# emanuele-artioli/elvis

Measured on AMD Instinct MI355X. Metric: restored 1080p frames/sec, SinSR 4x path (ELVIS v2 Downsample), higher is better.
Workload: dtype f16; 1 GPU; 30-frame 1920x1080 synthetic clip per GPU, ELVIS v2 Downsample (SinSR 4x), block 8, levels 0-3, weights seed 0 (random init), quantize=True; frames_per_gpu=30, parallelism=single GPU, gn_fused_into_conv=True, frames_per_invocation=15

## Files before the change

elvis_amd/csrc/conv.hip:

```cpp
#include "conv_kernels.inc"
#include "conv_ws.inc"
#include <string.h>

__attribute__((visibility("hidden"))) int elvis_conv_launch_f32_(const void* conv_args, int halo, int tco, int id, hipStream_t stream, void* query);
__attribute__((visibility("hidden"))) int elvis_conv_pack_x3p_(const float* w_oihw, void* packed, int cout, int ctot, int nkc, int n_co_tiles,
                                                              int tco, int taps, hipStream_t stream);

#include <atomic>
static std::atomic<int> g_no_halo{0};
static bool no_halo() { return g_no_halo.load(std::memory_order_relaxed) > 0; }
extern "C" int elvis_conv_debug_set(const char* key, int value) {
    ELVIS_REQUIRE(key, "elvis_conv_debug_set: null key");
    if (!strcmp(key, "no_halo")) { g_no_halo.store(value, std::memory_order_relaxed); return ELVIS_OK; }
    ELVIS_REQUIRE(false, "elvis_conv_debug_set: unknown key '%s'", key);
}

static void conv_geom(const elvis_conv_desc* d, int* nkc1, int* nkc, int* co_pad) {
    int kc = kc_of(d);
    *nkc1 = (d->cin + kc - 1) / kc;
    *nkc = *nkc1 + (d->cin2 > 0 ? (d->cin2 + kc - 1) / kc : 0);
    TileCfg t = choose_tile(d->cout);
    *co_pad = ((d->cout + t.tco - 1) / t.tco) * t.tco;
}

extern "C" size_t elvis_conv_packed_weight_bytes(const elvis_conv_desc* d) {
    if (!d || d->cin <= 0 || d->cout <= 0) return 0;
    int nkc1, nkc, co_pad;
    conv_geom(d, &nkc1, &nkc, &co_pad);
    return (size_t)d->ksize * d->ksize * nkc * co_pad * (x3_planar_fmt(d) ? 128 : 64);
}

extern "C" int elvis_conv_pack_weights(const elvis_conv_desc* d, const float* w_oihw, void* packed,
                                       elvis_stream_t stream) {
    int rc = validate(d);
    if (rc) return rc;
    ELVIS_REQUIRE(w_oihw && packed, "elvis_conv_pack_weights: null pointer");
    int nkc1, nkc, co_pad;
    conv_geom(d, &nkc1, &nkc, &co_pad);
    if (x3_planar_fmt(d)) {
        const int tco = choose_tile(d->cout).tco;
        return elvis_conv_pack_x3p_(w_oihw, packed, d->cout, d->cin + d->cin2, nkc, co_pad / tco, tco, d->ksize * d->ksize, (hipStream_t)stream);
    }
    int KC = kc_elems(d->dtype);
    long long total = (long long)d->ksize * d->ksize * nkc * co_pad * KC;
    int grid = (int)((total + 255) / 256);
    int ctot = d->cin + d->cin2;
    const int tco_ = choose_tile(d->cout).tco, wco = tco_ >= 64 ? 4 : tco_ / 16;
    if (d->dtype == ELVIS_F16)
        hipLaunchKernelGGL(pack_weights_kernel<half_t>, dim3(grid), dim3(256), 0, (hipStream_t)stream, w_oihw,
                           (half_t*)packed, d->cout, ctot, d->ksize, nkc, co_pad, KC, total, wco);
    else
        hipLaunchKernelGGL(pack_weights_kernel<float>, dim3(grid), dim3(256), 0, (hipStream_t)stream, w_oihw,
                           (float*)packed, d->cout, ctot, d->ksize, nkc, co_pad, KC, total, wco, d->dtype == ELVIS_F32X3 ? 1 : 0);
    ELVIS_CHECK_LAUNCH("elvis_conv_pack_weights");
    return ELVIS_OK;
}

static bool x3_eligible(const elvis_conv_desc* d) {
    if (!(d->dtype == ELVIS_F32X3 && halo_eligible(d) && !no_halo() && choose_tile(d->cout).tco >= 64)) return false;
    return !x3_planar_fmt(d) || x3_planar_run(d);
}
extern "C" int elvis_conv_x3_eligible(const elvis_conv_desc* d) {
    if (!d || validate(d)) return 0;
    return x3_eligible(d) ? 1 : 0;
}

enum class ConvPath { WS, HALO, IGEMM };
static ConvPath conv_path(const elvis_conv_desc* d, bool has_residual, bool has_stats) {
    if (no_halo()) return ConvPath::IGEMM;
    if (ws_shape_ok(d) && !has_residual && !has_stats) return ConvPath::WS;
    return halo_eligible(d) ? ConvPath::HALO : ConvPath::IGEMM;
}

static int conv_walk(const elvis_conv_desc* d, ConvPath path, const ConvArgs& a, hipStream_t stream, ConvPick* query) {
    const TileCfg t = choose_tile(d->cout);
    const bool f16 = d->dtype == ELVIS_F16;
    if (path == ConvPath::WS) return dispatch_ws(a, t.tco, stream, query);
    if (path == ConvPath::IGEMM) return f16 ? dispatch<half_t>(a, t.id, stream, query) : elvis_conv_launch_f32_(&a, 0, t.tco, t.id, stream, query);
    if (!f16) return elvis_conv_launch_f32_(&a, 1, t.tco, t.id, stream, query);
    switch (t.tco) {
        case 128: return launch_halo<half_t, 128>(a, stream, query);
        case 64: return launch_halo<half_t, 64>(a, stream, query);
        case 32: return launch_halo<half_t, 32>(a, stream, query);
        default: return launch_halo<half_t, 16>(a, stream, query);
    }
}

static int conv_plan(const elvis_conv_desc* d, ConvPath path, ConvArgs& a, ConvPick& pick) {
    a.n = d->n; a.h = d->h; a.w_in = d->w;
    a.cin = d->cin; a.cin_pitch = d->cin_pitch; a.cin2 = d->cin2; a.cin2_pitch = d->cin2_pitch;
    a.cout = d->cout; a.cout_pitch = d->cout_pitch;
    a.ksize = d->ksize; a.stride = d->stride; a.pad = d->pad_before; a.upsample = d->upsample;
    a.ho = d->ho; a.wo = d->wo; a.act = d->act; a.prologue = d->prologue;
    conv_geom(d, &a.nkc1, &a.nkc, &a.co_pad);
    TileCfg t = choose_tile(d->cout);
    a.M = (long long)d->n * d->ho * d->wo;
    a.n_co_tiles = a.co_pad / t.tco;
    a.n_px_tiles = (a.M + t.tpx - 1) / t.tpx;
    const bool s2d = d->ksize == 2 && d->subpixel == ELVIS_CONV_S2D;
    const bool subpix = d->ksize == 2 && !s2d;
    a.sub = d->ksize == 2;
    a.par_a = subpix ? (d->subpixel - 1) >> 1 : 0;
    a.par_b = subpix ? (d->subpixel - 1) & 1 : 0;
    a.ostr = subpix ? 2 : 1;
    a.pad2y = subpix ? 1 - a.par_a : (s2d ? d->pad_before : 0);
    a.pad2x = subpix ? 1 - a.par_b : (s2d ? d->pad_before : 0);
    a.s2d = s2d ? 1 : 0;
    a.istr = s2d ? 2 : 1;
    a.nkc_c = s2d ? d->cin / 4 / kc_of(d) : 0x3fffffff;
    a.wfull = d->w;
    if (s2d) {
        a.h = d->ho;
        a.w_in = d->wo;
    }
    a.x3 = d->dtype == ELVIS_F32X3 ? (x3_planar_run(d) ? 2 : 1) : 0;
    a.two = (halo_two(d) || halo_g1(d)) ? 1 : 0;
    a.tall = (halo_two(d) && halo_tall(d)) ? 1 : 0;
    int rc = conv_walk(d, path, a, nullptr, &pick);
    if (rc) return rc;
    a.tiles_x = ((subpix ? d->w : d->wo) + HALO_TX - 1) / HALO_TX;
    a.tiles_y = pick.ty > 0 ? ((subpix ? d->h : d->ho) + pick.ty - 1) / pick.ty : 0;
    a.strip = HALO_STRIP < a.tiles_x ? HALO_STRIP : 0;
    a.strip_full = a.strip > 0 ? a.tiles_x / a.strip : 0;
    return ELVIS_OK;
}

extern "C" int elvis_conv_stats_tiles(const elvis_conv_desc* d) {
    if (!d || !halo_eligible(d)) return 0;
    ConvArgs a{};
    ConvPick pick{};
    if (conv_plan(d, ConvPath::HALO, a, pick)) return 0;
    return d->n * a.tiles_y * a.tiles_x;
}

extern "C" int elvis_conv_kernel_name_for_call(const elvis_conv_desc* d, int has_residual, int has_stats, char* buf, size_t n) {
    int rc = validate(d);
    if (rc) return rc;
    ELVIS_REQUIRE(buf && n > 0, "elvis_conv_kernel_name: null buffer");
    ConvArgs a{};
    ConvPick pick{};
    rc = conv_plan(d, conv_path(d, has_residual != 0, has_stats != 0), a, pick);
    if (rc) return rc;
    snprintf(buf, n, "%s", pick.name);
    return ELVIS_OK;
}

extern "C" int elvis_conv_kernel_name(const elvis_conv_desc* d, char* buf, size_t n) {
    return elvis_conv_kernel_name_for_call(d, 0, 0, buf, n);
}

extern "C" int elvis_conv2d(const elvis_conv_desc* d, const void* x, const void* x2, const void* w_packed,
                            const float* bias, const void* residual, int residual_pitch, const float* pa,
                            const float* pb, void* out, float* stats, elvis_stream_t stream) {
    int rc = validate(d);
    if (rc) return rc;
    ELVIS_REQUIRE(x && w_packed && out, "elvis_conv2d: null pointer");
    ELVIS_REQUIRE(d->cin2 == 0 || x2, "elvis_conv2d: cin2 > 0 but x2 is null");
    ELVIS_REQUIRE(!d->prologue || (pa && pb), "elvis_conv2d: prologue requested without pa/pb");
    ELVIS_REQUIRE(d->dtype != ELVIS_F32X3 || x3_eligible(d),
                  "elvis_conv2d: this shape has no compensated-f16 kernel (elvis_conv_x3_eligible): run it as ELVIS_F32");
    ELVIS_REQUIRE(!residual || residual_pitch >= d->cout, "elvis_conv2d: bad residual pitch");
    ELVIS_REQUIRE(((uintptr_t)x | (uintptr_t)(x2 ? x2 : x) | (uintptr_t)w_packed | (uintptr_t)out) % 16 == 0,
                  "elvis_conv2d: pointers must be 16-byte aligned");
    const ConvPath path = conv_path(d, residual != nullptr, stats != nullptr);
    ELVIS_REQUIRE(path != ConvPath::IGEMM || !stats, "elvis_conv2d: fused statistics need a 3x3/stride-1 conv with cout >= 64 (query elvis_conv_stats_tiles)");
    ELVIS_REQUIRE(path == ConvPath::IGEMM || (long long)d->n * d->h * d->w < 0x7fffffffLL, "conv: input too large for 32-bit pixel indices");
    ConvArgs a{};
    ConvPick pick{};
    rc = conv_plan(d, path, a, pick);
    if (rc) return rc;
    a.x = x; a.x2 = x2; a.w = w_packed; a.bias = bias; a.res = residual; a.pa = pa; a.pb = pb; a.out = out;
    a.res_pitch = residual_pitch; a.stats = stats;
    return conv_walk(d, path, a, (hipStream_t)stream, nullptr);
}
```

elvis_amd/csrc/conv_kernels.inc:

```
#pragma once
#include "common.h"

#ifndef ELVIS_CONV_HOOKS
#define ELVIS_STAGE(x) x
#define ELVIS_STAGE_W(x) x
#define ELVIS_STAGE_H(x) x
#define ELVIS_SETPRIO(x)
#define ELVIS_BARRIER() __syncthreads()
#define ELVIS_HOOK_SKIP_STORE(tv)
#define ELVIS_HOOK_STAMP_BEGIN
#define ELVIS_HOOK_STAMP_LOOP
#define ELVIS_HOOK_STAMP_EPILOGUE
#define ELVIS_HOOK_STAMP_END
#endif

namespace {

struct ConvArgs {
    const void* x;
    const void* x2;
    const void* w;
    const float* bias;
    const void* res;
    const float* pa;
// ... 486 lines not shown
    int h_src[H_PER];
    unsigned h_ok = 0;
#pragma unroll
    for (int i = 0; i < H_PER; ++i) {
        int chunk = tid + i * NT;
        int pix = chunk >> 2;
        int hy = pix / HX, hx = pix - hy * HX;
        int gy = oy0 + hy - pad_y, gx = ox0 + hx - pad_x;
        bool ok = chunk < HCH && gy >= 0 && gy < lh && gx >= 0 && gx < lw;
        int sy = p.upsample ? (gy >> 1) : gy, sx = p.upsample ? (gx >> 1) : gx;
        h_src[i] = ok ? ((nimg * p.h + sy) * p.istr * p.w_in + sx) * p.istr : 0;
        h_ok |= (ok ? 1u : 0u) << i;
    }
    const bool halo_inside = oy0 - pad_y >= 0 && oy0 - pad_y + HY <= lh && ox0 - pad_x >= 0 && ox0 - pad_x + HX <= lw &&
                             (p.cin % KC) == 0 && (p.cin2 % KC) == 0 && p.cin_pitch >= p.nkc1 * KC && !(KS == 2 && p.s2d);
    const int q4 = tid & 3;
    const int nkc = p.nkc;
    const int nrows = nkc * KS;

    constexpr int HA = (H_PER + 1) / 2;
    uint4 hreg[H_PER];

    int wl_off[W_PER];
#pragma unroll
    for (int i = 0; i < W_PER; ++i) {
        int chunk = tid + i * NT;
        wl_off[i] = lds_row_off(chunk >> 2, chunk & 3);
    }

    auto chunk_c0 = [&](int kc, int& pixoff) -> int {
        pixoff = 0;
        if (KS == 2 && p.s2d) {
            const int ph = kc / p.nkc_c;
            pixoff = (ph >> 1) * p.wfull + (ph & 1);
            return (kc - ph * p.nkc_c) * KC + q4 * VEC;
        }
        return (kc >= p.nkc1 ? kc - p.nkc1 : kc) * KC + q4 * VEC;
    };
    auto halo_load = [&](int kc, int i0, int i1, bool live = true) {
        const bool second = kc >= p.nkc1;
        const char* xsrc = (const char*)(second ? p.x2 : p.x);
        const int pitch = second ? p.cin2_pitch : p.cin_pitch;
        int pixoff;
        const int c0 = chunk_c0(kc, pixoff);
        const int c0c = c0 < pitch ? c0 : 0;
        const long long lv = live ? (long long)sizeof(T) : 0;
#pragma unroll
        for (int i = i0; i < i1; ++i)
            hreg[i] = *reinterpret_cast<const uint4*>(xsrc + ((long long)(h_src[i] + pixoff) * pitch + c0c) * lv);
    };
    auto halo_store = [&](int kc, int buf, int i0, int i1) {
        const bool second = kc >= p.nkc1;
        const int pitch = second ? p.cin2_pitch : p.cin_pitch;
        int pixoff_;
        const int c0 = chunk_c0(kc, pixoff_);
        const bool ch_ok = c0 < pitch;
        char* dst = halo + buf * HALO_BYTES;
        float la[VEC], lb[VEC];
        if (PRO) {
            const float* tp = ptab + (kc * 4 + q4) * 2 * VEC;
#pragma unroll
            for (int e = 0; e < VEC; e += 4) {
                float4v a4 = *reinterpret_cast<const float4v*>(tp + e);
                float4v b4 = *reinterpret_cast<const float4v*>(tp + VEC + e);
#pragma unroll
                for (int k = 0; k < 4; ++k) { la[e + k] = a4[k]; lb[e + k] = b4[k]; }
            }
        }
#pragma unroll
        for (int i = i0; i < i1; ++i) {
            uint4 v = hreg[i];
            if constexpr (PSC) {
                const float K = -1.4426950408889634f;
                v.x = prologue_dword_f16(v.x, la[0], la[1], lb[0], lb[1], K);
                v.y = prologue_dword_f16(v.y, la[2], la[3], lb[2], lb[3], K);
                v.z = prologue_dword_f16(v.z, la[4], la[5], lb[4], lb[5], K);
                v.w = prologue_dword_f16(v.w, la[6], la[7], lb[6], lb[7], K);
            } else if (PRO) {
                v = prologue_apply<T>(v, la, lb);
            }
            if constexpr (X3) v = x3_pair4(v);
            if (!halo_inside) {
                const bool keep = ch_ok && ((h_ok >> i) & 1u);
                v.x = keep ? v.x : 0u; v.y = keep ? v.y : 0u; v.z = keep ? v.z : 0u; v.w = keep ? v.w : 0u;
            }
            int chunk = tid + i * NT;
            if ((i + 1) * NT <= HCH || chunk < HCH)
                *reinterpret_cast<uint4*>(dst + lds_row_off(chunk >> 2, chunk & 3)) = v;
        }
    };
    auto halo_act = [&](int kc, int slot, int half) {
        constexpr int HV = VEC / 2;
        const float* tp = ptab + (kc * 4 + q4) * 2 * VEC + half * HV;
        float a[HV], b[HV];
#pragma unroll
        for (int e = 0; e < HV; e += 2) {
            float2 a2 = *reinterpret_cast<const float2*>(tp + e);
            float2 b2 = *reinterpret_cast<const float2*>(tp + VEC + e);
            a[e] = a2.x; a[e + 1] = a2.y; b[e] = b2.x; b[e + 1] = b2.y;
        }
        uint2 v = half ? make_uint2(hreg[slot].z, hreg[slot].w) : make_uint2(hreg[slot].x, hreg[slot].y);
        v = prologue_apply_half(v, a, b, T());
        if (half) { hreg[slot].z = v.x; hreg[slot].w = v.y; } else { hreg[slot].x = v.x; hreg[slot].y = v.y; }
    };
    auto halo_write = [&](int kc, int buf, int slot) {
        const bool second = kc >= p.nkc1;
        const int pitch = second ? p.cin2_pitch : p.cin_pitch;
        int pixoff_;
        const int c0 = chunk_c0(kc, pixoff_);
        const bool keep = c0 < pitch && ((h_ok >> slot) & 1u);
        uint4 v = hreg[slot];
        if constexpr (X3) v = x3_pair4(v);
        v.x = keep ? v.x : 0u; v.y = keep ? v.y : 0u; v.z = keep ? v.z : 0u; v.w = keep ? v.w : 0u;
        int chunk = tid + slot * NT;
        if ((slot + 1) * NT <= HCH || chunk < HCH)
            *reinterpret_cast<uint4*>(halo + buf * HALO_BYTES + lds_row_off(chunk >> 2, chunk & 3)) = v;
    };
    static_assert(W_PER <= 2, "weight staging holds at most two 16-byte chunks per thread per tap");
    constexpr bool W_FULL0 = W_CHUNKS >= NT, W_FULL1 = W_PER == 2 && W_CHUNKS >= 2 * NT;
    const bool w_ok0 = W_FULL0 || tid < W_CHUNKS, w_ok1 = W_PER == 2 && (W_FULL1 || tid + NT < W_CHUNKS);
    uint4 wr00 = {}, wr01 = {}, wr10 = {}, wr11 = {}, wr20 = {}, wr21 = {};
    auto w_load = [&](int r) {
        r = r < nrows ? r : nrows - 1;
        int kc = r / KS, dy = r - kc * KS;
        const long long tap_stride = (long long)nkc * p.co_pad * 64;
        const char* wsrc = (const char*)p.w + ((long long)(dy * KS * nkc + kc) * p.co_pad + co0) * 64;
        const int o0 = (w_ok0 ? tid : 0) * 16, o1 = (w_ok1 ? tid + NT : 0) * 16;
        wr00 = *reinterpret_cast<const uint4*>(wsrc + o0);
        if (W_PER == 2) wr01 = *reinterpret_cast<const uint4*>(wsrc + o1);
        if (KS >= 2) {
            wr10 = *reinterpret_cast<const uint4*>(wsrc + tap_stride + o0);
            if (W_PER == 2) wr11 = *reinterpret_cast<const uint4*>(wsrc + tap_stride + o1);
        }
        if (KS == 3) {
            wr20 = *reinterpret_cast<const uint4*>(wsrc + 2 * tap_stride + o0);
            if (W_PER == 2) wr21 = *reinterpret_cast<const uint4*>(wsrc + 2 * tap_stride + o1);
        }
    };
    auto w_store = [&](int slot) {
        char* dst = wring + slot * W_BYTES;
        if (w_ok0) *reinterpret_cast<uint4*>(dst + wl_off[0]) = wr00;
        if (W_PER == 2 && w_ok1) *reinterpret_cast<uint4*>(dst + wl_off[W_PER - 1]) = wr01;
        if (KS >= 2) {
            if (w_ok0) *reinterpret_cast<uint4*>(dst + W_TAP_BYTES + wl_off[0]) = wr10;
            if (W_PER == 2 && w_ok1) *reinterpret_cast<uint4*>(dst + W_TAP_BYTES + wl_off[W_PER - 1]) = wr11;
        }
        if (KS == 3) {
            if (w_ok0) *reinterpret_cast<uint4*>(dst + 2 * W_TAP_BYTES + wl_off[0]) = wr20;
            if (W_PER == 2 && w_ok1) *reinterpret_cast<uint4*>(dst + 2 * W_TAP_BYTES + wl_off[W_PER - 1]) = wr21;
        }
    };
    const int wave_u = __builtin_amdgcn_readfirstlane(tid >> 6);
    const unsigned lds_base = __builtin_amdgcn_readfirstlane((unsigned)(uintptr_t)(lds_ptr_t)smem);
    auto w_glds = [&](int r, int slot) {
        r = r < nrows ? r : nrows - 1;
        int kc = r / KS, dy = r - kc * KS;
        const long long tap_stride = (long long)nkc * p.co_pad * 64;
        const char* wsrc = (const char*)p.w + ((long long)(dy * KS * nkc + kc) * p.co_pad + co0) * 64;
#pragma unroll
        for (int t = 0; t < KS; ++t)
#pragma unroll
            for (int i = 0; i < W_PER; ++i)
            {
                unsigned keep;
                const unsigned dst = lds_base + (unsigned)((wring - smem) + slot * W_BYTES + t * W_TAP_BYTES + (i * NT + wave_u * 64) * 16);
                const char* src = wsrc + t * tap_stride + wl_off[i];
                asm volatile("s_mov_b32 %0, m0\n\ts_mov_b32 m0, %2\n\ts_nop 0\n\tglobal_load_lds_dwordx4 %1, off\n\ts_mov_b32 m0, %0"
                             : "=&s"(keep) : "v"(src), "s"(dst) : "memory");
            }
    };
    auto w_glds_wait = [&]() { asm volatile("s_waitcnt vmcnt(0)" ::: "memory"); };

    float4v acc[WCO][WPX];
    auto acc_zero = [&]() {
#pragma unroll
        for (int i = 0; i < WCO; ++i)
#pragma unroll
            for (int j = 0; j < WPX; ++j) acc[i][j] = (float4v){0.f, 0.f, 0.f, 0.f};
    };

    const int lane_off = lds_row_off(lane & 15, lane >> 4);
    const int lq = lane >> 4, lr = lane & 15;

    constexpr bool EARLY = !G1 && !(NT == 256 && TCO == 64 && TY == 16) && !(NT == 256 && TCO == 128 && KS == 2);
    if constexpr (EARLY) {
        halo_load(0, 0, H_PER);
        if constexpr (WDMA) w_glds(0, 0); else w_load(0);
    }
    const bool fold = !ACT;
    const bool vec4 = (p.cout & 3) == 0 && (p.res_pitch & 3) == 0;
    bool co_ok[WCO];
#pragma unroll
    for (int i = 0; i < WCO; ++i) co_ok[i] = co0 + w_co * (16 * WCO) + lq * (4 * WCO) + i * 4 < p.cout;
    auto load_bias = [&](float (&bv)[WCO][4]) {
#pragma unroll
        for (int i = 0; i < WCO; ++i) {
            const int co = co0 + w_co * (16 * WCO) + lq * (4 * WCO) + i * 4;
#pragma unroll
            for (int r = 0; r < 4; ++r) bv[i][r] = 0.f;
            if (p.bias) {
                const float* bp = p.bias + (co_ok[i] ? co : 0);
#pragma unroll
                for (int r = 0; r < 4; ++r) bv[i][r] = bp[r];
            }
        }
    };
    constexpr bool WIDE16 = WCO == 4 && sizeof(T) == 2;
    const bool wide16 = WIDE16 && vec4 && (p.cout & 15) == 0 && (p.res_pitch & 7) == 0 && (p.cout_pitch & 7) == 0 &&
                        (((uintptr_t)p.res | (uintptr_t)p.out) & 15) == 0;
    if (fold && vec4) {
        float bv[WCO][4];
        load_bias(bv);
        if (p.res) {
#pragma unroll
            for (int j = 0; j < WPX; ++j) {
                const int oy = oy0 + w_px * ROWS + (j >> 1), ox = ox0 + (j & 1) * 16 + lr;
                const bool pix_ok = KS == 2 ? (oy < p.h && ox < p.w_in) : (oy < p.ho && ox < p.wo);
                const long long m = KS == 2 ? ((long long)nimg * p.ho + p.ostr * oy + p.par_a) * p.wo + p.ostr * ox + p.par_b
                                            : ((long long)nimg * p.ho + oy) * p.wo + ox;
                const long long mc = pix_ok ? m : 0;
                if constexpr (WIDE16) {
                    if (wide16) {
                        const T* rp = (const T*)p.res + mc * p.res_pitch + (co_ok[0] ? co0 + w_co * 64 + lq * 16 : 0);
                        acc[0][j] = __builtin_bit_cast(float4v, *reinterpret_cast<const uint4*>(rp));
                        acc[2][j] = __builtin_bit_cast(float4v, *reinterpret_cast<const uint4*>(rp + 8));
                        continue;
                    }
                }
#pragma unroll
                for (int i = 0; i < WCO; ++i) {
                    const int co = co0 + w_co * (16 * WCO) + lq * (4 * WCO) + i * 4;
                    const T* rp = (const T*)p.res + mc * p.res_pitch + (co_ok[i] ? co : 0);
                    if constexpr (sizeof(T) == 2) {
                        half4 rv = *reinterpret_cast<const half4*>(rp);
#pragma unroll
                        for (int r = 0; r < 4; ++r) acc[i][j][r] = bv[i][r] + (float)rv[r];
                    } else {
                        float4v rv = *reinterpret_cast<const float4v*>(rp);
#pragma unroll
                        for (int r = 0; r < 4; ++r) acc[i][j][r] = bv[i][r] + rv[r];
                    }
                }
            }
        } else {
#pragma unroll
            for (int j = 0; j < WPX; ++j)
#pragma unroll
                for (int i = 0; i < WCO; ++i)
#pragma unroll
                    for (int r = 0; r < 4; ++r) acc[i][j][r] = bv[i][r];
        }
    } else if (fold && (p.res || p.bias)) {
        acc_zero();
#pragma unroll
        for (int j = 0; j < WPX; ++j) {
            const int oy = oy0 + w_px * ROWS + (j >> 1), ox = ox0 + (j & 1) * 16 + lr;
            const bool pix_ok = KS == 2 ? (oy < p.h && ox < p.w_in) : (oy < p.ho && ox < p.wo);
            const long long m = KS == 2 ? ((long long)nimg * p.ho + p.ostr * oy + p.par_a) * p.wo + p.ostr * ox + p.par_b
                                        : ((long long)nimg * p.ho + oy) * p.wo + ox;
#pragma unroll
            for (int i = 0; i < WCO; ++i) {
                const int co = co0 + w_co * (16 * WCO) + lq * (4 * WCO) + i * 4;
                if (!pix_ok || co >= p.cout) continue;
                const int nv = p.cout - co < 4 ? p.cout - co : 4;
                float v[4] = {0.f, 0.f, 0.f, 0.f};
                if (p.bias) {
#pragma unroll
                    for (int r = 0; r < 4; ++r)
                        if (r < nv) v[r] = p.bias[co + r];
                }
                if (p.res) {
                    const T* rp = (const T*)p.res + m * p.res_pitch + co;
                    if (nv == 4) {
                        if constexpr (sizeof(T) == 2) {
                            half4 rv = *reinterpret_cast<const half4*>(rp);
#pragma unroll
                            for (int r = 0; r < 4; ++r) v[r] += (float)rv[r];
                        } else {
                            float4v rv = *reinterpret_cast<const float4v*>(rp);
#pragma unroll
                            for (int r = 0; r < 4; ++r) v[r] += rv[r];
                        }
                    } else {
                        for (int r = 0; r < nv; ++r) v[r] += to_f(rp[r]);
                    }
                }
#pragma unroll
                for (int r = 0; r < 4; ++r) acc[i][j][r] = v[r];
            }
        }
    } else {
        acc_zero();
    }

    auto res_convert = [&]() {
        if constexpr (WIDE16) {
            if (fold && wide16 && p.res) {
                float bv[WCO][4];
                load_bias(bv);
#pragma unroll
                for (int j = 0; j < WPX; ++j) {
                    const uint4 rlo = __builtin_bit_cast(uint4, acc[0][j]), rhi = __builtin_bit_cast(uint4, acc[2][j]);
                    const unsigned rw[8] = {rlo.x, rlo.y, rlo.z, rlo.w, rhi.x, rhi.y, rhi.z, rhi.w};
#pragma unroll
                    for (int d = 0; d < 8; ++d) {
                        float f0, f1;
                        asm("v_fma_mix_f32 %0, %1, 1.0, %2 op_sel:[0,0,0] op_sel_hi:[1,0,0]" : "=v"(f0) : "v"(rw[d]), "v"(bv[d >> 1][(d & 1) * 2]));
                        asm("v_fma_mix_f32 %0, %1, 1.0, %2 op_sel:[1,0,0] op_sel_hi:[1,0,0]" : "=v"(f1) : "v"(rw[d]), "v"(bv[d >> 1][(d & 1) * 2 + 1]));
                        acc[d >> 1][j][(d & 1) * 2] = f0;
                        acc[d >> 1][j][(d & 1) * 2 + 1] = f1;
                    }
                }
            }
        }
    };
    if constexpr (G1) {
        constexpr int STAGE = HALO_BYTES + W_TAP_BYTES;
        constexpr int L = H_PER + W_PER;
        static_assert(HCH % NT == 0 && W_CHUNKS % NT == 0, "G1 stages are whole 1 KiB wave pieces");
        const int swz_t = ((tid >> 4) & 1) << 1;
        const int wave_u1 = __builtin_amdgcn_readfirstlane(tid >> 6);
        const unsigned lds0 = __builtin_amdgcn_readfirstlane((unsigned)(uintptr_t)(lds_ptr_t)smem);
        auto g1_dma = [&](const char* src, unsigned dst) {
            unsigned keep;
            asm volatile("s_mov_b32 %0, m0\n\ts_mov_b32 m0, %2\n\ts_nop 0\n\tglobal_load_lds_dwordx4 %1, off\n\ts_mov_b32 m0, %0"
                         : "=&s"(keep) : "v"(src), "s"(dst) : "memory");
        };
        auto g1_issue = [&](int kc) {
            const int slot = kc % G1_NST;
            const bool second = kc >= p.nkc1;
            const char* xsrc = (const char*)(second ? p.x2 : p.x);
            const long long pitch = second ? p.cin2_pitch : p.cin_pitch;
            const int c0 = (second ? kc - p.nkc1 : kc) * KC + ((q4 ^ swz_t) * VEC);
#pragma unroll
            for (int i = 0; i < H_PER; ++i)
                g1_dma(xsrc + ((long long)h_src[i] * pitch + c0) * (long long)sizeof(T),
                       lds0 + (unsigned)(slot * STAGE + (i * NT + wave_u1 * 64) * 16));
            const char* wsrc = (const char*)p.w + ((long long)kc * p.co_pad + co0) * 64;
#pragma unroll
            for (int i = 0; i < W_PER; ++i)
                g1_dma(wsrc + wl_off[i], lds0 + (unsigned)(slot * STAGE + HALO_BYTES + (i * NT + wave_u1 * 64) * 16));
        };
#pragma unroll
        for (int s = 0; s < G1_NST - 1; ++s)
            if (s < nkc) g1_issue(s);
        res_convert();
        const int pp0 = (w_px * ROWS) * HX + lr;
        int bb[4][2];
#pragma unroll
        for (int r = 0; r < 4; ++r)
#pragma unroll
            for (int e = 0; e < 2; ++e) {
                int carry = ((pp0 & 3) + r) >> 2;
                int bit = ((pp0 >> 2) & 1) ^ carry ^ e;
                bb[r][e] = pp0 * 64 + ((lq ^ (bit << 1)) << 4);
            }
        const int a_off = HALO_BYTES + w_co * WCO * 1024 + lane_off;
        ELVIS_HOOK_STAMP_LOOP
        for (int kc = 0; kc < nkc; ++kc) {
            if (kc + G1_NST - 2 < nkc) asm volatile("s_waitcnt vmcnt(%0)" :: "n"((G1_NST - 2) * L) : "memory");
            else asm volatile("s_waitcnt vmcnt(0)" ::: "memory");
            __syncthreads();
            if (kc + G1_NST - 1 < nkc) g1_issue(kc + G1_NST - 1);
            const int sb = (kc % G1_NST) * STAGE;
            frag_t fa[WCO];
#pragma unroll
            for (int i = 0; i < WCO; ++i) fa[i] = lds_frag<frag_t>(smem + sb + a_off + i * 1024);
#pragma unroll
            for (int j = 0; j < WPX; ++j) {
                const int C = (j >> 1) * HX + (j & 1) * 16;
                frag_t fb = lds_frag<frag_t>(smem + sb + bb[C & 3][(C >> 2) & 1] + C * 64);
#pragma unroll
                for (int i = 0; i < WCO; ++i) mma_tile_x<X3>(acc[i][j], fa[i], fb);
            }
        }
        __syncthreads();
    } else {
    if constexpr (!EARLY && !G1) {
        halo_load(0, 0, H_PER);
        if constexpr (WDMA) w_glds(0, 0); else w_load(0);
    }
    if (PRO) {
        const int ctot = p.cin + p.cin2;
        for (int t2 = tid; t2 < nkc * 4 * VEC; t2 += NT) {
            int kc = t2 / (4 * VEC), r = t2 - kc * 4 * VEC;
            bool second = kc >= p.nkc1;
            int cl = (second ? kc - p.nkc1 : kc) * KC + r;
            bool in = cl < (second ? p.cin2 : p.cin);
            long long g = (long long)nimg * ctot + (second ? p.cin : 0) + (in ? cl : 0);
            int q = r / VEC, e = r - q * VEC;
            const float psc = PSC ? -1.4426950408889634f : 1.0f;
            ptab[(kc * 4 + q) * 2 * VEC + e] = in ? psc * p.pa[g] : 0.0f;
            ptab[(kc * 4 + q) * 2 * VEC + VEC + e] = in ? psc * p.pb[g] : 0.0f;
        }
        __syncthreads();
    }
    halo_store(0, 0, 0, H_PER);
    res_convert();
    if constexpr (WDMA) {
        w_glds_wait();
    } else {
        w_store(0);
        w_load(1);
    }
    __syncthreads();

    ELVIS_HOOK_STAMP_LOOP
    const int pp0 = (w_px * ROWS) * HX + lr;
    int bb[4][2];
#pragma unroll
    for (int r = 0; r < 4; ++r)
#pragma unroll
        for (int e = 0; e < 2; ++e) {
            int carry = ((pp0 & 3) + r) >> 2;
            int bit = ((pp0 >> 2) & 1) ^ carry ^ e;
            bb[r][e] = pp0 * 64 + ((lq ^ (bit << 1)) << 4);
        }
    const int a_off = w_co * WCO * 1024 + lane_off;

#define ELVIS_ROW_STEP(DY)                                                                             \
    {                                                                                                  \
        const int rslot = TWO ? ((r0 + DY) & 1) : DY;                                                  \
        if constexpr (WDMA) {                                                                          \
            ELVIS_STAGE_W(w_glds(r0 + DY + 1, rslot ^ 1);)                                             \
        } else {                                                                                       \
            ELVIS_STAGE(w_store(TWO ? (rslot ^ 1) : (DY + 1) % NSLOT);)                                \
            ELVIS_STAGE(w_load(r0 + DY + 2);)                                                          \
        }                                                                                              \
        ELVIS_STAGE_H(if (DY == 0) halo_load(kcn, 0, PRO ? H_PER : HA, kc + 1 < nkc);)                 \
        ELVIS_STAGE_H(if (DY == 1 && !PRO) halo_load(kcn, HA, H_PER, kc + 1 < nkc);)                   \
        if constexpr (TWO) {                                                                           \
              \
            const char* wsb = wring + rslot * W_BYTES + a_off;                                         \
            frag_t fa[2][WCO], fb[2];                                                                  \
            _Pragma("unroll") for (int i = 0; i < WCO; ++i)                                            \
                fa[0][i] = lds_frag<frag_t>(wsb + i * 1024);                           \
            {                                                                                          \
                const int C = DY * HX;                                                                 \
                fb[0] = lds_frag<frag_t>(smem + bb[C & 3][(C >> 2) & 1] + C * 64);     \
            }                                                                                          \
            ELVIS_SETPRIO(1);                                                                          \
            _Pragma("unroll") for (int s = 0; s < KS * WPX; ++s) {                                     \
                const int dx = s / WPX, j = s - dx * WPX;                                              \
                if (s + 1 < KS * WPX) {                                                                \
                    const int ndx = (s + 1) / WPX, nj = (s + 1) - ndx * WPX;                           \
                    const int C = ((nj >> 1) + DY) * HX + (nj & 1) * 16 + ndx;                         \
                    fb[(s + 1) & 1] = lds_frag<frag_t>(smem + bb[C & 3][(C >> 2) & 1] + C * 64); \
                }                                                                                      \
                if (dx + 1 < KS && j < WCO)                                                            \
                    fa[(dx + 1) & 1][j] = lds_frag<frag_t>(wsb + (dx + 1) * W_TAP_BYTES + j * 1024); \
                _Pragma("unroll") for (int i = 0; i < WCO; ++i) mma_tile_x<X3>(acc[i][j], fa[dx & 1][i], fb[s & 1]); \
            }                                                                                          \
            ELVIS_SETPRIO(0);                                                                          \
            __builtin_amdgcn_sched_group_barrier(0x100, WCO + 1, 0);                                   \
            _Pragma("unroll") for (int s = 0; s < KS * WPX; ++s) {                                     \
                if ((s % WPX) < WCO && s / WPX + 1 < KS) __builtin_amdgcn_sched_group_barrier(0x100, 2, 0); \
                else if (s + 1 < KS * WPX) __builtin_amdgcn_sched_group_barrier(0x100, 1, 0);          \
                __builtin_amdgcn_sched_group_barrier(0x008, WCO, 0);                                   \
            }                                                                                          \
        } else {                                                                                       \
        _Pragma("unroll") for (int dx = 0; dx < KS; ++dx) {                                            \
            const char* ws = wring + rslot * W_BYTES + dx * W_TAP_BYTES + a_off;                       \
            frag_t fa[WCO];                                                                            \
            _Pragma("unroll") for (int i = 0; i < WCO; ++i)                                            \
                fa[i] = lds_frag<frag_t>(ws + i * 1024);                               \
            _Pragma("unroll") for (int j = 0; j < WPX; ++j) {                                          \
                const int C = ((j >> 1) + DY) * HX + (j & 1) * 16 + dx;                                \
                frag_t fb = lds_frag<frag_t>(smem + bb[C & 3][(C >> 2) & 1] + C * 64); \
                _Pragma("unroll") for (int i = 0; i < WCO; ++i) mma_tile_x<X3>(acc[i][j], fa[i], fb);        \
                               \
                if (PRO && DY >= 1 && j == WPX / 2 - 1) {                                              \
                    _Pragma("unroll") for (int pi = 0; pi < 2 * H_PER; ++pi)                           \
                        if (pi * 6 / (2 * H_PER) == (DY - 1) * 3 + dx) {                               \
                            ELVIS_STAGE(halo_act(kcn, pi / 2, pi & 1);)                                \
                            if ((pi & 1) && !TWO) { ELVIS_STAGE(halo_write(kcn, (kc + 1) & 1, pi / 2);) } \
                        }                                                                              \
                }                                                                                      \
            }                                                                                          \
                            \
            if (PRO && DY >= 1 && !TWO) {                                                              \
                _Pragma("unroll") for (int g = 0; g < WCO * WPX; ++g) {                                \
                    __builtin_amdgcn_sched_group_barrier(0x008, 1, 0);                                 \
                    __builtin_amdgcn_sched_group_barrier(0x002, 3, 0);                                 \
                }                                                                                      \
            }                                                                                          \
        }                                                                                              \
        }                                                                                              \
        ELVIS_STAGE(if (DY == 0 && !PRO && !TWO) halo_store(kcn, (kc + 1) & 1, 0, HA);)                \
        ELVIS_STAGE(if (DY == 1 && !PRO && !TWO) halo_store(kcn, (kc + 1) & 1, HA, H_PER);)            \
        if constexpr (WDMA) {                                                                          \
                            \
            constexpr int YOUNGER = DY == 0 ? (PRO ? H_PER : HA) : (DY == 1 && !PRO) ? H_PER - HA : 0;           \
            ELVIS_STAGE_W(asm volatile("s_waitcnt vmcnt(%0)" :: "n"(YOUNGER) : "memory");)            \
        }                                                                                              \
        ELVIS_BARRIER();                                                                               \
    }
    for (int kc = 0; kc < nkc; ++kc) {
        const int r0 = kc * KS;
        const int kcn = kc + 1 < nkc ? kc + 1 : kc;
        if constexpr (KS == 3) {
            ELVIS_ROW_STEP(0)
            ELVIS_ROW_STEP(1)
            ELVIS_ROW_STEP(2)
        } else if constexpr (KS == 2) {
            ELVIS_ROW_STEP(0)
            ELVIS_ROW_STEP(1)
        } else {
            const int slot = kc % 3;
            w_store((kc + 1) % 3);
            w_load(kc + 2);
            halo_load(kcn, 0, H_PER);
            const char* ws = wring + slot * W_BYTES + a_off;
            frag_t fa[WCO];
#pragma unroll
            for (int i = 0; i < WCO; ++i) fa[i] = lds_frag<frag_t>(ws + i * 1024);
#pragma unroll
            for (int j = 0; j < WPX; ++j) {
                const int C = (j >> 1) * HX + (j & 1) * 16;
                frag_t fb = lds_frag<frag_t>(smem + bb[C & 3][(C >> 2) & 1] + C * 64);
#pragma unroll
                for (int i = 0; i < WCO; ++i) mma_tile_x<X3>(acc[i][j], fa[i], fb);
            }
            halo_store(kcn, (kc + 1) & 1, 0, H_PER);
            __syncthreads();
        }
        if constexpr (TWO) {
            ELVIS_STAGE_H(if (kc + 1 < nkc) {
                halo_store(kcn, 0, 0, H_PER);
            })
            __syncthreads();
        } else {
            const int delta = (kc & 1) ? -HALO_BYTES : HALO_BYTES;
#pragma unroll
            for (int r = 0; r < 4; ++r) {
                bb[r][0] += delta;
                bb[r][1] += delta;
            }
        }
    }
#undef ELVIS_ROW_STEP
    }
    ELVIS_HOOK_STAMP_EPILOGUE

    float st[WCO][4], sq[WCO][4];
#pragma unroll
    for (int i = 0; i < WCO; ++i)
#pragma unroll
        for (int r = 0; r < 4; ++r) st[i][r] = sq[i][r] = 0.f;
    const int cgrp = lq * 4;
    constexpr bool LEAN = TWO && WIDE16 && !ACT && !X3 && (WPX % 2 == 0);
    bool lean_done = false;
    if constexpr (LEAN) {
        const bool interior = wide16 && co0 + TCO <= p.cout &&
                              (KS == 2 ? (oy0 + TY <= p.h && ox0 + TX <= p.w_in) : (oy0 + TY <= p.ho && ox0 + TX <= p.wo));
        if (interior) {
            typedef _Float16 half2v __attribute__((ext_vector_type(2)));
            const half2v ones = {(_Float16)1.f, (_Float16)1.f};
            unsigned prev[8];
#pragma unroll
            for (int j = 0; j < WPX; ++j) {
                const int oy = oy0 + w_px * ROWS + (j >> 1), ox = ox0 + (j & 1) * 16 + lr;
                const long long m = KS == 2 ? ((long long)nimg * p.ho + p.ostr * oy + p.par_a) * p.wo + p.ostr * ox + p.par_b
                                            : ((long long)nimg * p.ho + oy) * p.wo + ox;
                unsigned cur[8];
#pragma unroll
                for (int k = 0; k < 8; ++k) {
                    const half2v h2 = {(_Float16)acc[k >> 1][j][(k & 1) * 2], (_Float16)acc[k >> 1][j][(k & 1) * 2 + 1]};
                    cur[k] = __builtin_bit_cast(unsigned, h2);
                }
                T* op = (T*)p.out + m * p.cout_pitch + co0 + w_co * 64 + lq * 16;
                *reinterpret_cast<uint4*>(op) = make_uint4(cur[0], cur[1], cur[2], cur[3]);
                *reinterpret_cast<uint4*>(op + 8) = make_uint4(cur[4], cur[5], cur[6], cur[7]);
                if (p.stats) {
                    if (j & 1) {
#pragma unroll
                        for (int k = 0; k < 8; ++k) {
                            const half2v e = __builtin_bit_cast(half2v, __builtin_amdgcn_perm(cur[k], prev[k], 0x05040100u));
                            const half2v o = __builtin_bit_cast(half2v, __builtin_amdgcn_perm(cur[k], prev[k], 0x07060302u));
                            const int i = k >> 1, r = (k & 1) * 2;
                            st[i][r] = __builtin_amdgcn_fdot2(e, ones, st[i][r], false);
                            sq[i][r] = __builtin_amdgcn_fdot2(e, e, sq[i][r], false);
                            st[i][r + 1] = __builtin_amdgcn_fdot2(o, ones, st[i][r + 1], false);
                            sq[i][r + 1] = __builtin_amdgcn_fdot2(o, o, sq[i][r + 1], false);
                        }
                    } else {
#pragma unroll
                        for (int k = 0; k < 8; ++k) prev[k] = cur[k];
                    }
                }
            }
            lean_done = true;
        }
    }
    if (lean_done) {
    } else if (vec4) {
        float bv[WCO][4];
        if constexpr (ACT) load_bias(bv);
#pragma unroll
        for (int j = 0; j < WPX; ++j) {
            const int oy = oy0 + w_px * ROWS + (j >> 1), ox = ox0 + (j & 1) * 16 + lr;
            const bool pix_ok = KS == 2 ? (oy < p.h && ox < p.w_in) : (oy < p.ho && ox < p.wo);
            const long long m = KS == 2 ? ((long long)nimg * p.ho + p.ostr * oy + p.par_a) * p.wo + p.ostr * ox + p.par_b
                                        : ((long long)nimg * p.ho + oy) * p.wo + ox;
            const long long mc = pix_ok ? m : 0;
            T wv[WCO][4];
#pragma unroll
            for (int i = 0; i < WCO; ++i) {
                const int co = co0 + w_co * (16 * WCO) + cgrp * WCO + i * 4;
                const bool ok = pix_ok && co_ok[i];
                float v[4] = {acc[i][j][0], acc[i][j][1], acc[i][j][2], acc[i][j][3]};
                if constexpr (ACT) {
#pragma unroll
                    for (int r = 0; r < 4; ++r) v[r] += bv[i][r];
                    if (p.act == 1) {
#pragma unroll
                        for (int r = 0; r < 4; ++r) v[r] = gelu_erf_f(v[r]);
                    } else if (p.act == 2) {
#pragma unroll
                        for (int r = 0; r < 4; ++r) v[r] = v[r] / (1.0f + expf(-v[r]));
                    } else {
#pragma unroll
                        for (int r = 0; r < 4; ++r) v[r] = fmaxf(v[r], 0.0f);
                    }
                    if (p.res) {
                        const T* rp = (const T*)p.res + mc * p.res_pitch + (co_ok[i] ? co : 0);
                        if constexpr (sizeof(T) == 2) {
                            half4 rv = *reinterpret_cast<const half4*>(rp);
#pragma unroll
                            for (int r = 0; r < 4; ++r) v[r] += (float)rv[r];
                        } else {
                            float4v rv = *reinterpret_cast<const float4v*>(rp);
#pragma unroll
                            for (int r = 0; r < 4; ++r) v[r] += rv[r];
                        }
                    }
                }
                T tv[4];
#pragma unroll
                for (int r = 0; r < 4; ++r) tv[r] = from_f<T>(v[r]);
                T* op = (T*)p.out + m * p.cout_pitch + co;
                ELVIS_HOOK_SKIP_STORE(tv)
                if (ok && !wide16) {
                    if constexpr (sizeof(T) == 2) {
                        half4 hv = {tv[0], tv[1], tv[2], tv[3]};
                        *reinterpret_cast<half4*>(op) = hv;
                    } else {
                        *reinterpret_cast<float4v*>(op) = (float4v){tv[0], tv[1], tv[2], tv[3]};
                    }
                } else if (pix_ok && !co_ok[i] && co < p.cout_pitch) {
                    if constexpr (sizeof(T) == 2) *reinterpret_cast<half4*>(op) = (half4){(half_t)0, (half_t)0, (half_t)0, (half_t)0};
                    else *reinterpret_cast<float4v*>(op) = (float4v){0.f, 0.f, 0.f, 0.f};
                }
// ... 179 lines not shown

constexpr int halo_tile_rows(int ks, bool pro, int tco, int nt, bool tall) {
    if (nt == 256) return ks == 1 ? (tco == 128 ? G1_TY128 : G1_TY64) : tall ? HALO_TY2_TALL : HALO_TY2;
    if (ks == 3 && pro && tco == 128) return HALO_TY_PRO128;
    return (pro || ks == 1 || tco <= 32) ? HALO_TY_PRO : HALO_TY;
}
constexpr int x3p_tile_rows(int tco) { return tco == 128 ? X3P_TY128 : X3P_TY64; }

constexpr size_t halo_tile_bytes(int ty, int ks) { return (size_t)(ty + ks - 1) * (HALO_TX + ks - 1) * 64; }
constexpr size_t halo_lds_bytes(int ks, int tco, int ty, int nt, int pro_chunks, int kc = 32) {
    const bool two = nt == 256;
    const size_t fixed = (two && ks == 1) ? (tco == 64 ? G1_NST64 : G1_NST128) * ((size_t)ty * HALO_TX * 64 + (size_t)tco * 64)
                                          : (two ? 1 : 2) * halo_tile_bytes(ty, ks) + ((two || ks == 2) ? 2 : 3) * ks * (size_t)tco * 64;
    return fixed + (size_t)pro_chunks * kc * 2 * sizeof(float);
}

inline bool halo_tall(const elvis_conv_desc* d) {
    return d->ksize == 3 && choose_tile(d->cout).tco == 64 && (d->prologue || d->cin + d->cin2 <= 32) &&
           (long long)d->ho * d->wo >= 128 * 1024;
}
inline int kc_elems(int dtype) { return dtype == ELVIS_F16 ? 32 : 16; }
inline int conv_nkc32(const elvis_conv_desc* d) { return (d->cin + 31) / 32 + (d->cin2 > 0 ? (d->cin2 + 31) / 32 : 0); }
inline bool x3_planar_fmt(const elvis_conv_desc* d) {
    if (d->dtype != ELVIS_F32X3 || choose_tile(d->cout).tco < 64 || d->cout % 4) return false;
    if (d->ksize == 2) return d->subpixel != ELVIS_CONV_S2D || d->cin % 128 == 0;
    return d->ksize == 3 && (d->cin2 == 0 || d->cin % 32 == 0);
}
inline bool x3_planar_run(const elvis_conv_desc* d) {
    if (!x3_planar_fmt(d)) return false;
    if (d->ksize == 2) return true;
    return d->stride == 1 && d->pad_before == 1 && !d->upsample && d->ho == d->h && d->wo == d->w;
}
inline int kc_of(const elvis_conv_desc* d) { return x3_planar_fmt(d) ? 32 : kc_elems(d->dtype); }
inline bool halo_two(const elvis_conv_desc* d) {
    const int tco = choose_tile(d->cout).tco, ks = d->ksize;
    if ((ks != 3 && ks != 2) || d->dtype != ELVIS_F16 || tco < 64) return false;
    const int ty = halo_tile_rows(ks, d->prologue != 0, tco, 256, halo_tall(d));
    return halo_lds_bytes(ks, tco, ty, 256, d->prologue ? conv_nkc32(d) : 0) <= 80 * 1024;
}
static_assert(halo_lds_bytes(3, 128, HALO_TY2, 256, 0) == 70912 && halo_lds_bytes(3, 64, HALO_TY2_TALL, 256, 0) <= 80 * 1024,
              "a conv without the prologue must fit the 256-thread kernel: at most 70 912 bytes (launch_halo relies on it)");
inline bool halo_g1(const elvis_conv_desc* d) {
    return d->ksize == 1 && d->dtype == ELVIS_F16 && choose_tile(d->cout).tco >= 64 && d->cin % 32 == 0 &&
           d->cin2 % 32 == 0;
}

int validate(const elvis_conv_desc* d) {
    ELVIS_REQUIRE(d, "conv: null descriptor");
    ELVIS_REQUIRE(d->dtype == ELVIS_F32 || d->dtype == ELVIS_F16 || d->dtype == ELVIS_F32X3, "conv: bad dtype %d", d->dtype);
    ELVIS_REQUIRE(d->n > 0 && d->h > 0 && d->w > 0 && d->cin > 0 && d->cout > 0 && d->ho > 0 && d->wo > 0,
                  "conv: bad shape n=%d h=%d w=%d cin=%d cout=%d ho=%d wo=%d", d->n, d->h, d->w, d->cin, d->cout, d->ho, d->wo);
    ELVIS_REQUIRE(d->ksize == 1 || d->ksize == 3 || (d->ksize == 2 && d->subpixel >= 1 && d->subpixel <= 5),
                  "conv: ksize must be 1 or 3, or 2 with subpixel = 1 + parity / 5 (got ksize %d, subpixel %d)", d->ksize, d->subpixel);
    const bool s2d = d->ksize == 2 && d->subpixel == ELVIS_CONV_S2D;
    if (d->ksize == 2 && !s2d)
        ELVIS_REQUIRE(d->stride == 1 && !d->upsample && !d->prologue && d->ho == 2 * d->h && d->wo == 2 * d->w,
                      "conv: a sub-pixel parity conv maps h x w to 2h x 2w, stride 1, no prologue");
    if (s2d)
        ELVIS_REQUIRE(!d->upsample && !d->prologue && d->cin2 == 0 && d->h == 2 * d->ho && d->w == 2 * d->wo && d->cout >= 32 &&
                          (d->pad_before == 0 || d->pad_before == 1) &&
                          ((d->dtype == ELVIS_F16 && d->cin % 128 == 0) || (d->dtype == ELVIS_F32X3 && d->cin % 64 == 0 && d->cout >= 64)),
                      "conv: the space-to-depth stride-2 form maps 2ho x 2wo to ho x wo, f16 (cin = 4 x a multiple of 32, cout >= 32) or "
                      "compensated fp32 (cin = 4 x a multiple of 16, cout >= 64), pad_before 0 or 1");
    ELVIS_REQUIRE(d->stride == 1 || d->stride == 2, "conv: stride must be 1 or 2");
    ELVIS_REQUIRE(d->cin_pitch >= (s2d ? d->cin / 4 : d->cin) && d->cin_pitch % 8 == 0, "conv: cin_pitch %d must be >= cin %d and a multiple of 8", d->cin_pitch, d->cin);
    ELVIS_REQUIRE(d->cout_pitch >= d->cout && d->cout_pitch % 4 == 0, "conv: cout_pitch %d invalid for cout %d", d->cout_pitch, d->cout);
    int kc = kc_of(d);
    if (d->cin2 > 0) {
        ELVIS_REQUIRE(d->cin % kc == 0, "conv: with a second input, cin (%d) must be a multiple of %d", d->cin, kc);
        ELVIS_REQUIRE(d->cin2_pitch >= d->cin2 && d->cin2_pitch % 8 == 0, "conv: bad cin2_pitch");
    }
    int lh = d->upsample ? 2 * d->h : d->h, lw = d->upsample ? 2 * d->w : d->w;
    ELVIS_REQUIRE(d->ksize == 2 ||
                  ((long long)(d->ho - 1) * d->stride - d->pad_before < lh && (long long)(d->wo - 1) * d->stride - d->pad_before < lw),
                  "conv: output %dx%d does not fit input %dx%d (stride %d)", d->ho, d->wo, lh, lw, d->stride);
    return ELVIS_OK;
}

template <typename T, int WCO, int WPX, int NW_CO, int NW_PX>
int launch(const ConvArgs& a, hipStream_t stream, ConvPick* query) {
    static const ElvisKernelName name("conv_igemm_kernel<%s,%d,%d,%d,%d>", sizeof(T) == 2 ? "half" : "float", WCO, WPX, NW_CO, NW_PX);
    if (query) return query->set(name.s, 0);
    constexpr int TCO = 16 * WCO * NW_CO, TPX = 16 * WPX * NW_PX;
    size_t lds = 2 * (size_t)(TCO + TPX) * 64;
    long long nblk = (long long)a.n_co_tiles * a.n_px_tiles;
    ELVIS_REQUIRE(nblk < 0x7fffffffLL, "conv: grid too large");
    hipLaunchKernelGGL((conv_igemm_kernel<T, WCO, WPX, NW_CO, NW_PX>), dim3((unsigned)nblk), dim3(64 * NW_CO * NW_PX),
                       lds, stream, a);
    ELVIS_CHECK_LAUNCH("elvis_conv2d");
    elvis_note_launch(name.s);
    return ELVIS_OK;
}

template <typename T, int TCO, bool PRO, int KS, int NT = 512, bool ACT = false, bool TALL = false, bool X3 = false>
int launch_halo_p(const ConvArgs& a, hipStream_t stream, ConvPick* query) {
    if constexpr (!ACT) {
        if (a.act != 0) return launch_halo_p<T, TCO, PRO, KS, NT, true, TALL, X3>(a, stream, query);
    }
    if constexpr (!X3 && sizeof(T) == 4 && NT == 512 && TCO >= 64) {
        if (a.x3) return launch_halo_p<T, TCO, PRO, KS, NT, ACT, TALL, true>(a, stream, query);
    }
    constexpr int TY = halo_tile_rows(KS, PRO, TCO, NT, TALL);
    static const ElvisKernelName name = X3 ? ElvisKernelName("conv3x3_halo_x3_kernel<%d,%d,%s,%d,%s>", TCO, TY, tf(PRO), KS, tf(ACT))
                                    : ElvisKernelName("conv3x3_halo_kernel<%s,%d,%d,%d,%s,%d,%s>", sizeof(T) == 2 ? "half" : "float", TCO, NT, TY, tf(PRO), KS, tf(ACT));
    if (query) return query->set(name.s, TY);
    const void* fn = nullptr;
    if constexpr (X3) fn = (const void*)conv3x3_halo_x3_kernel<TCO, TY, PRO, KS, ACT>;
    else fn = (const void*)conv3x3_halo_kernel<T, TCO, NT, TY, PRO, KS, ACT>;
    const size_t lds = halo_lds_bytes(KS, TCO, TY, NT, PRO ? a.nkc : 0, 4 * DT<T>::VEC);
    ELVIS_REQUIRE(lds <= 160 * 1024, "conv3x3_halo: %zu bytes of LDS needed (too many input channels)", lds);
    static ElvisLdsOptIn opt_in;
    if (int rc = elvis_lds_opt_in(fn, opt_in, elvis_device_slot(), "conv3x3_halo: cannot reserve %zu bytes of LDS", lds)) return rc;
    long long nblk = (long long)a.n_co_tiles * a.tiles_x * a.tiles_y * a.n;
    ELVIS_REQUIRE(nblk < 0x7fffffffLL, "conv: grid too large");
    if constexpr (X3) hipLaunchKernelGGL((conv3x3_halo_x3_kernel<TCO, TY, PRO, KS, ACT>), dim3((unsigned)nblk), dim3(NT), lds, stream, a);
    else hipLaunchKernelGGL((conv3x3_halo_kernel<T, TCO, NT, TY, PRO, KS, ACT>), dim3((unsigned)nblk), dim3(NT), lds, stream, a);
    ELVIS_CHECK_LAUNCH("elvis_conv2d(halo)");
    elvis_note_launch(name.s);
    return ELVIS_OK;
}

template <typename T, int TCO> int launch_halo(const ConvArgs& a, hipStream_t stream, ConvPick* query) {
    if constexpr (TCO >= 64 && sizeof(T) == 2) {
        if (a.two && a.ksize == 1) return launch_halo_p<T, TCO, false, 1, 256>(a, stream, query);
    }
    if (a.ksize == 1) return launch_halo_p<T, TCO, false, 1>(a, stream, query);
    if constexpr (TCO >= 64 && sizeof(T) == 2) {
        if (a.two && a.ksize == 2) return launch_halo_p<T, TCO, false, 2, 256>(a, stream, query);
        if constexpr (TCO == 64) {
            if (a.two && a.tall && a.ksize == 3)
                return a.prologue ? launch_halo_p<T, TCO, true, 3, 256, false, true>(a, stream, query)
                                  : launch_halo_p<T, TCO, false, 3, 256, false, true>(a, stream, query);
        }
        if (a.two) return a.prologue ? launch_halo_p<T, TCO, true, 3, 256>(a, stream, query) : launch_halo_p<T, TCO, false, 3, 256>(a, stream, query);
        ELVIS_REQUIRE(a.ksize == 3 && a.prologue, "conv3x3_halo: a conv without the prologue must fit the 256-thread kernel");
        return launch_halo_p<T, TCO, true, 3>(a, stream, query);
    } else {
        if (a.ksize == 2) return launch_halo_p<T, TCO, false, 2>(a, stream, query);
        return a.prologue ? launch_halo_p<T, TCO, true, 3>(a, stream, query) : launch_halo_p<T, TCO, false, 3>(a, stream, query);
    }
}

template <typename T> int dispatch(const ConvArgs& a, int id, hipStream_t stream, ConvPick* query) {
    switch (id) {
        case 0: return launch<T, 4, 4, 2, 2>(a, stream, query);
        case 1: return launch<T, 4, 2, 1, 4>(a, stream, query);
        case 2: return launch<T, 2, 4, 1, 4>(a, stream, query);
        default: return launch<T, 1, 4, 1, 4>(a, stream, query);
    }
}

template <typename T>
__global__ void pack_weights_kernel(const float* __restrict__ w, T* __restrict__ out, int cout, int ctot, int ks,
                                    int nkc, int co_pad, int KC, long long total, int wco, int pairs = 0) {
    long long i = (long long)blockIdx.x * blockDim.x + threadIdx.x;
    if (i >= total) return;
    int k = (int)(i % KC);
    long long t = i / KC;
    int row = (int)(t % co_pad);
    const int G = 16 * wco;
    const int rho = row % G, fi = rho / 16, q = (rho % 16) / 4, rr = rho % 4;
    int co = (row / G) * G + q * 4 * wco + fi * 4 + rr;
    t /= co_pad;
    int kc = (int)(t % nkc);
    int tap = (int)(t / nkc);
    int ci = kc * KC + k;
    float v = 0.f;
    if (co < cout && ci < ctot) v = w[((long long)co * ctot + ci) * ks * ks + tap];
    if constexpr (sizeof(T) == 4) {
        if (pairs) {
            reinterpret_cast<unsigned*>(out)[i] = x3_pair(v);
            return;
        }
    }
    out[i] = from_f<T>(v);
}

}
```

Baseline: 32.31 frames/s.

## Skip all-zero space-to-depth conv taps using a packed weight tap mask

When packing weights for space-to-depth 2x2 convolutions, the pack kernel now records a bitmask of which (phase, tap) combinations hold any nonzero weight and stores it in a trailer after the packed weights. The halo conv kernel reads this mask and skips the weight DMA and MMA work for taps that are entirely zero, using a single-tap path when only one tap of a row is live. This targets wasted load and matrix work in the downsample convolutions, where the space-to-depth rearrangement leaves many taps zero. The cost is extra branching and a second single-tap code path in the inner loop, which may add register pressure, plus a debug switch to turn the skipping off.

```diff
diff --git a/elvis_amd/csrc/conv.hip b/elvis_amd/csrc/conv.hip
--- a/elvis_amd/csrc/conv.hip
+++ b/elvis_amd/csrc/conv.hip
@@ -7,11 +7,13 @@
                                                               int tco, int taps, hipStream_t stream);
 
 #include <atomic>
-static std::atomic<int> g_no_halo{0};
+static std::atomic<int> g_no_halo{0}, g_s2d_all_taps{0};
 static bool no_halo() { return g_no_halo.load(std::memory_order_relaxed) > 0; }
+static bool s2d_all_taps() { return g_s2d_all_taps.load(std::memory_order_relaxed) > 0; }
 extern "C" int elvis_conv_debug_set(const char* key, int value) {
     ELVIS_REQUIRE(key, "elvis_conv_debug_set: null key");
     if (!strcmp(key, "no_halo")) { g_no_halo.store(value, std::memory_order_relaxed); return ELVIS_OK; }
+    if (!strcmp(key, "s2d_all_taps")) { g_s2d_all_taps.store(value, std::memory_order_relaxed); return ELVIS_OK; }
     ELVIS_REQUIRE(false, "elvis_conv_debug_set: unknown key '%s'", key);
 }
 
@@ -23,11 +25,17 @@
     *co_pad = ((d->cout + t.tco - 1) / t.tco) * t.tco;
 }
 
-extern "C" size_t elvis_conv_packed_weight_bytes(const elvis_conv_desc* d) {
-    if (!d || d->cin <= 0 || d->cout <= 0) return 0;
+constexpr size_t S2D_TRAILER_BYTES = 64;
+static bool s2d_mask_fmt(const elvis_conv_desc* d) { return d->ksize == 2 && d->subpixel == ELVIS_CONV_S2D && !x3_planar_fmt(d); }
+static size_t packed_body_bytes(const elvis_conv_desc* d) {
     int nkc1, nkc, co_pad;
     conv_geom(d, &nkc1, &nkc, &co_pad);
     return (size_t)d->ksize * d->ksize * nkc * co_pad * (x3_planar_fmt(d) ? 128 : 64);
+}
+
+extern "C" size_t elvis_conv_packed_weight_bytes(const elvis_conv_desc* d) {
+    if (!d || d->cin <= 0 || d->cout <= 0) return 0;
+    return packed_body_bytes(d) + (s2d_mask_fmt(d) ? S2D_TRAILER_BYTES : 0);
 }
 
 extern "C" int elvis_conv_pack_weights(const elvis_conv_desc* d, const float* w_oihw, void* packed,
@@ -46,12 +54,18 @@
     int grid = (int)((total + 255) / 256);
     int ctot = d->cin + d->cin2;
     const int tco_ = choose_tile(d->cout).tco, wco = tco_ >= 64 ? 4 : tco_ / 16;
+    unsigned* tapmask = nullptr;
+    if (s2d_mask_fmt(d)) {
+        tapmask = reinterpret_cast<unsigned*>((char*)packed + packed_body_bytes(d));
+        ELVIS_REQUIRE(hipMemsetAsync(tapmask, 0, S2D_TRAILER_BYTES, (hipStream_t)stream) == hipSuccess, "elvis_conv_pack_weights: cannot clear the mask trailer");
+    }
+    const int nkc_c = tapmask ? nkc / 4 : 1;
     if (d->dtype == ELVIS_F16)
         hipLaunchKernelGGL(pack_weights_kernel<half_t>, dim3(grid), dim3(256), 0, (hipStream_t)stream, w_oihw,
-                           (half_t*)packed, d->cout, ctot, d->ksize, nkc, co_pad, KC, total, wco);
+                           (half_t*)packed, d->cout, ctot, d->ksize, nkc, co_pad, KC, total, wco, 0, tapmask, nkc_c);
     else
         hipLaunchKernelGGL(pack_weights_kernel<float>, dim3(grid), dim3(256), 0, (hipStream_t)stream, w_oihw,
-                           (float*)packed, d->cout, ctot, d->ksize, nkc, co_pad, KC, total, wco, d->dtype == ELVIS_F32X3 ? 1 : 0);
+                           (float*)packed, d->cout, ctot, d->ksize, nkc, co_pad, KC, total, wco, d->dtype == ELVIS_F32X3 ? 1 : 0, tapmask, nkc_c);
     ELVIS_CHECK_LAUNCH("elvis_conv_pack_weights");
     return ELVIS_OK;
 }
@@ -171,5 +185,6 @@
     if (rc) return rc;
     a.x = x; a.x2 = x2; a.w = w_packed; a.bias = bias; a.res = residual; a.pa = pa; a.pb = pb; a.out = out;
     a.res_pitch = residual_pitch; a.stats = stats;
+    if (s2d_mask_fmt(d) && d->dtype == ELVIS_F16 && !s2d_all_taps()) a.s2d = 2;
     return conv_walk(d, path, a, (hipStream_t)stream, nullptr);
 }
diff --git a/elvis_amd/csrc/conv_kernels.inc b/elvis_amd/csrc/conv_kernels.inc
--- a/elvis_amd/csrc/conv_kernels.inc
+++ b/elvis_amd/csrc/conv_kernels.inc
@@ -662,7 +662,7 @@
     };
     const int wave_u = __builtin_amdgcn_readfirstlane(tid >> 6);
     const unsigned lds_base = __builtin_amdgcn_readfirstlane((unsigned)(uintptr_t)(lds_ptr_t)smem);
-    auto w_glds = [&](int r, int slot) {
+    auto w_glds = [&](int r, int slot, unsigned taps = 3u) {
         r = r < nrows ? r : nrows - 1;
         int kc = r / KS, dy = r - kc * KS;
         const long long tap_stride = (long long)nkc * p.co_pad * 64;
@@ -672,6 +672,9 @@
 #pragma unroll
             for (int i = 0; i < W_PER; ++i)
             {
+                if constexpr (KS == 2) {
+                    if (!((taps >> t) & 1u)) continue;
+                }
                 unsigned keep;
                 const unsigned dst = lds_base + (unsigned)((wring - smem) + slot * W_BYTES + t * W_TAP_BYTES + (i * NT + wave_u * 64) * 16);
                 const char* src = wsrc + t * tap_stride + wl_off[i];
@@ -932,14 +935,38 @@
     {                                                                                                  \
         const int rslot = TWO ? ((r0 + DY) & 1) : DY;                                                  \
         if constexpr (WDMA) {                                                                          \
-            ELVIS_STAGE_W(w_glds(r0 + DY + 1, rslot ^ 1);)                                             \
+            ELVIS_STAGE_W(w_glds(r0 + DY + 1, rslot ^ 1, DY + 1 < KS ? (m4 >> 2) & 3u : m4n & 3u);)    \
         } else {                                                                                       \
             ELVIS_STAGE(w_store(TWO ? (rslot ^ 1) : (DY + 1) % NSLOT);)                                \
             ELVIS_STAGE(w_load(r0 + DY + 2);)                                                          \
         }                                                                                              \
         ELVIS_STAGE_H(if (DY == 0) halo_load(kcn, 0, PRO ? H_PER : HA, kc + 1 < nkc);)                 \
         ELVIS_STAGE_H(if (DY == 1 && !PRO) halo_load(kcn, HA, H_PER, kc + 1 < nkc);)                   \
+                                                       \
+        unsigned taps = 3u;                                                                            \
+        if constexpr (TWO && KS == 2) {                                                                \
+            taps = (m4 >> (2 * DY)) & 3u;                                                              \
+            _Pragma("unroll") for (int d = 0; d < 2; ++d)                                              \
+                if (taps == (1u << d)) {                                                               \
+                    const char* wsb = wring + rslot * W_BYTES + d * W_TAP_BYTES + a_off;               \
+                    frag_t fa[WCO], fb[2];                                                             \
+                    _Pragma("unroll") for (int i = 0; i < WCO; ++i)                                    \
+                        fa[i] = lds_frag<frag_t>(wsb + i * 1024);                                      \
+                    {                                                                                  \
+                        const int C = DY * HX + d;                                                     \
+                        fb[0] = lds_frag<frag_t>(smem + bb[C & 3][(C >> 2) & 1] + C * 64);             \
+                    }                                                                                  \
+                    _Pragma("unroll") for (int j = 0; j < WPX; ++j) {                                  \
+                        if (j + 1 < WPX) {                                                             \
+                            const int C = (((j + 1) >> 1) + DY) * HX + ((j + 1) & 1) * 16 + d;         \
+                            fb[(j + 1) & 1] = lds_frag<frag_t>(smem + bb[C & 3][(C >> 2) & 1] + C * 64); \
+                        }                                                                              \
+                        _Pragma("unroll") for (int i = 0; i < WCO; ++i) mma_tile_x<X3>(acc[i][j], fa[i], fb[j & 1]); \
+                    }                                                                                  \
+                }                                                                                      \
+        }                                                                                              \
         if constexpr (TWO) {                                                                           \
+            if (KS != 2 || taps == 3u) {                                                               \
               \
             const char* wsb = wring + rslot * W_BYTES + a_off;                                         \
             frag_t fa[2][WCO], fb[2];                                                                  \
@@ -967,6 +994,7 @@
                 if ((s % WPX) < WCO && s / WPX + 1 < KS) __builtin_amdgcn_sched_group_barrier(0x100, 2, 0); \
                 else if (s + 1 < KS * WPX) __builtin_amdgcn_sched_group_barrier(0x100, 1, 0);          \
                 __builtin_amdgcn_sched_group_barrier(0x008, WCO, 0);                                   \
+            }                                                                                          \
             }                                                                                          \
         } else {                                                                                       \
         _Pragma("unroll") for (int dx = 0; dx < KS; ++dx) {                                            \
@@ -1005,9 +1033,23 @@
         }                                                                                              \
         ELVIS_BARRIER();                                                                               \
     }
+    unsigned tmask = 0xffffu, m4 = 15u, m4n = 15u;
+    int ph_left = p.nkc_c;
+    if constexpr (TWO && KS == 2) {
+        if (p.s2d > 1) tmask = *reinterpret_cast<const unsigned*>((const char*)p.w + (long long)(KS * KS) * nkc * p.co_pad * 64);
+        m4n = tmask & 15u;
+    }
     for (int kc = 0; kc < nkc; ++kc) {
         const int r0 = kc * KS;
         const int kcn = kc + 1 < nkc ? kc + 1 : kc;
+        if constexpr (TWO && KS == 2) {
+            m4 = m4n;
+            if (--ph_left == 0) {
+                ph_left = p.nkc_c;
+                tmask >>= 4;
+            }
+            m4n = kc + 1 < nkc ? tmask & 15u : 15u;
+        }
         if constexpr (KS == 3) {
             ELVIS_ROW_STEP(0)
             ELVIS_ROW_STEP(1)
@@ -1493,7 +1535,8 @@
 
 template <typename T>
 __global__ void pack_weights_kernel(const float* __restrict__ w, T* __restrict__ out, int cout, int ctot, int ks,
-                                    int nkc, int co_pad, int KC, long long total, int wco, int pairs = 0) {
+                                    int nkc, int co_pad, int KC, long long total, int wco, int pairs = 0,
+                                    unsigned* __restrict__ tapmask = nullptr, int nkc_c = 1) {
     long long i = (long long)blockIdx.x * blockDim.x + threadIdx.x;
     if (i >= total) return;
     int k = (int)(i % KC);
@@ -1508,6 +1551,10 @@
     int ci = kc * KC + k;
     float v = 0.f;
     if (co < cout && ci < ctot) v = w[((long long)co * ctot + ci) * ks * ks + tap];
+    if (tapmask && !(to_f(from_f<T>(v)) == 0.f)) {
+        const unsigned bit = 1u << ((kc / nkc_c) * 4 + tap);
+        if (!(__atomic_load_n(tapmask, __ATOMIC_RELAXED) & bit)) atomicOr(tapmask, bit);
+    }
     if constexpr (sizeof(T) == 4) {
         if (pairs) {
             reinterpret_cast<unsigned*>(out)[i] = x3_pair(v);
```

Result: no change. 32.44 frames/s, median of 3 (+0.4%).
